# foolwood/SiamMask

Hardware: NVIDIA H100
Metric: search-region frames/sec (127/255 SiamMask-sharp) (higher is better)
Workload: dtype f16x3 (hi+lo split fp16 operands on wgmma, f32 accumulate; f32 CUDA-core xcorr/refine)

## Files before the change

siammask_b200/csrc/conv_gemm_sm90.cu:

```cuda
#include "common.cuh"
#include "ptx.cuh"

#include <cstdlib>
#include <cstring>
#include <mutex>
#include <unordered_map>

namespace smk {

namespace {

constexpr int BLOCK_M = 128;
constexpr int WG_ROWS = 64;
constexpr int CIN_GRAIN = 64;
constexpr int MMA_K = 16;
constexpr int SMEM_LIMIT = 227 * 1024;
constexpr int NUM_CONSUMER_WARPS = 8;
constexpr int NUM_THREADS = 128 + 32 * NUM_CONSUMER_WARPS;
constexpr int PRODUCER_REGS = 40;
constexpr int CONSUMER_REGS = 232;

template <int BLOCK_N, int NSPLIT>
struct Cfg {
  static constexpr int STAGING_BYTES = WG_ROWS * BLOCK_N * 4;
  static constexpr int RING_BYTES = SMEM_LIMIT - 2048 - 2 * STAGING_BYTES;
  static constexpr int stage_bytes(int bk) { return NSPLIT * (BLOCK_M + BLOCK_N) * bk * 2; }
  static constexpr int BLOCK_K = RING_BYTES / stage_bytes(64) >= 3 ? 64 : 32;
  static constexpr int SW = BLOCK_K * 2;
  static constexpr int A_TILE_BYTES = BLOCK_M * BLOCK_K * 2;
  static constexpr int B_TILE_BYTES = BLOCK_N * BLOCK_K * 2;
  static constexpr int STAGE_BYTES = NSPLIT * (A_TILE_BYTES + B_TILE_BYTES);
  static constexpr int RAW_STAGES = RING_BYTES / STAGE_BYTES;
  static constexpr int STAGES = RAW_STAGES > 6 ? 6 : RAW_STAGES;
  static constexpr int SMEM_BYTES = STAGES * STAGE_BYTES + 2 * STAGING_BYTES + 1024  + 256 ;
  static constexpr int ACC = BLOCK_N / 2;
  static constexpr int H_BOX = BLOCK_N < 64 ? BLOCK_N : 64;
  static constexpr int F_BOX = BLOCK_N < 32 ? BLOCK_N : 32;
  static constexpr int H_PLANE = WG_ROWS * BLOCK_N * 2;
  static_assert(STAGES >= 3, "pipeline needs at least three stages");
  static_assert(BLOCK_N % 16 == 0 && BLOCK_N >= 16 && BLOCK_N <= 128, "N tile (register accumulators)");
  static_assert(STAGE_BYTES % 1024 == 0 && B_TILE_BYTES % 1024 == 0, "stage parts stay 1024-aligned (swizzle atoms)");
  static_assert(SMEM_BYTES <= SMEM_LIMIT, "shared memory budget");
};

__device__ __forceinline__ int m_block(const GemmParams& p, int tile) {
  const int mb = tile / p.n_tiles;
  return p.reverse_m ? p.m_tiles - 1 - mb : mb;
}

template <int SPAN>
__device__ __forceinline__ uint32_t swizzle(uint32_t o) {
  return o ^ (((o >> 7) & (SPAN / 16 - 1)) << 4);
}

__device__ __forceinline__ void named_barrier_sync(int id, int threads) {
  asm volatile("bar.sync %0, %1;" ::"r"(id), "r"(threads) : "memory");
}

template <int BLOCK_N, int NSPLIT>
__global__ void __launch_bounds__(NUM_THREADS, 1) conv_gemm_kernel(const __grid_constant__ GemmParams p) {
  using C = Cfg<BLOCK_N, NSPLIT>;
  constexpr int STAGES = C::STAGES;
  constexpr int BLOCK_K = C::BLOCK_K;
  constexpr int A_TILE_BYTES = C::A_TILE_BYTES;

  extern __shared__ uint8_t smem_raw[];
  uint8_t* smem = smem_raw + ((1024u - (smem_u32(smem_raw) & 1023u)) & 1023u);
  uint8_t* staging = smem + STAGES * C::STAGE_BYTES;
  uint64_t* full_bar = reinterpret_cast<uint64_t*>(staging + 2 * C::STAGING_BYTES);
  uint64_t* empty_bar = full_bar + STAGES;
  uint64_t* free_bar = empty_bar + STAGES;
  uint64_t* res_bar = free_bar + 2;

  const int warp = __shfl_sync(0xffffffffu, (int)(threadIdx.x >> 5), 0);
  const int lane = threadIdx.x & 31;
  const int num_tiles = p.m_tiles * p.n_tiles;

  if (threadIdx.x == 0) {
    for (int i = 0; i < NSPLIT; ++i) {
      for (int sgi = 0; sgi < p.nseg; ++sgi) tma_prefetch_desc(&p.seg[sgi].tmA[i]);
      tma_prefetch_desc(&p.tmB[i]);
    }
    for (int s = 0; s < STAGES; ++s) {
      mbar_init(&full_bar[s], 1);
      mbar_init(&empty_bar[s], NUM_CONSUMER_WARPS);
    }
    for (int w = 0; w < 2; ++w) {
      mbar_init(&free_bar[w], 1);
      mbar_init(&res_bar[w], 1);
    }
    fence_barrier_init();
  }
  __syncthreads();

  if (warp < 4) {
    setmaxnreg_dec<PRODUCER_REGS>();
    if (warp != 0) return;
    const bool leader = elect_one();
    int stage = 0;
    uint32_t phase = 0;
    uint32_t iter = 0;
    for (int tile = blockIdx.x; tile < num_tiles; tile += gridDim.x, ++iter) {
      const int m0 = m_block(p, tile) * BLOCK_M;
      const int n0 = (tile % p.n_tiles) * BLOCK_N;
      const int q = m0 % p.Wo;
      const int t = m0 / p.Wo;
      const int pq = t % p.Ho;
      const int nb = t / p.Ho;
      for (int sgi = 0; sgi < p.nseg; ++sgi) {
        const GemmSegment& sg = p.seg[sgi];
        const int wb = q * sg.stride - sg.pad;
        const int hb = pq * sg.stride - sg.pad;
#pragma unroll 1
        for (int kb = 0; kb < sg.num_kb; ++kb) {
          mbar_wait(&empty_bar[stage], phase ^ 1);
          if (leader) mbar_arrive_expect_tx(&full_bar[stage], C::STAGE_BYTES);
          uint8_t* st = smem + stage * C::STAGE_BYTES;
          const int tap = kb / sg.cblks;
          const int c0 = (kb - tap * sg.cblks) * BLOCK_K;
#pragma unroll
          for (int s = 0; s < NSPLIT; ++s) {
            uint8_t* a_dst = st + s * A_TILE_BYTES;
            if (leader) {
              if (sg.mode == 0) {
                tma_load_2d(a_dst, &sg.tmA[s], &full_bar[stage], c0, m0);
              } else {
                const int r = tap / sg.KW;
                const int sx = tap - r * sg.KW;
                tma_load_im2col_4d(a_dst, &sg.tmA[s], &full_bar[stage], c0, wb, hb, nb,
                                   static_cast<uint16_t>(sx * sg.dil), static_cast<uint16_t>(r * sg.dil));
              }
              tma_load_2d(st + NSPLIT * A_TILE_BYTES + s * C::B_TILE_BYTES, &p.tmB[s], &full_bar[stage],
                          sg.b_col0 + kb * BLOCK_K, n0);
            }
          }
          __syncwarp();
          if (++stage == STAGES) { stage = 0; phase ^= 1; }
        }
      }
      if (p.has_res) {
#pragma unroll 1
        for (int w = 0; w < 2; ++w) {
          mbar_wait(&free_bar[w], iter & 1);
          const int r0 = m0 + w * WG_ROWS;
          if (leader) {
            mbar_arrive_expect_tx(&res_bar[w], r0 < p.M ? NSPLIT * C::H_PLANE : 0);
            if (r0 < p.M) {
              uint8_t* dst = staging + w * C::STAGING_BYTES;
#pragma unroll
              for (int s = 0; s < NSPLIT; ++s)
#pragma unroll
                for (int b = 0; b < BLOCK_N / C::H_BOX; ++b)
                  tma_load_2d(dst + s * C::H_PLANE + b * (WG_ROWS * C::H_BOX * 2), &p.tmR[s], &res_bar[w],
                              n0 + b * C::H_BOX, r0);
            }
          }
          __syncwarp();
        }
      }
    }
    return;
  }

  setmaxnreg_inc<CONSUMER_REGS>();
  const int wg = (warp >> 2) - 1;
  const int wl = warp & 3;
  const bool store_thread = wl == 0 && lane == 0;
  const Epilogue& ep = p.ep;
  const int HoWo = p.Ho * p.Wo;
  uint8_t* my_staging = staging + wg * C::STAGING_BYTES;
  float acc[C::ACC];
  float acc2[C::ACC];
  int stage = 0;
  uint32_t phase = 0;
  uint32_t iter = 0;
  for (int tile = blockIdx.x; tile < num_tiles; tile += gridDim.x, ++iter) {
#pragma unroll
    for (int i = 0; i < C::ACC; ++i) { acc[i] = 0.f; acc2[i] = 0.f; }
    int prev = -1;
    for (int sgi = 0; sgi < p.nseg; ++sgi) {
      const int nkb = p.seg[sgi].num_kb;
#pragma unroll 1
      for (int kb = 0; kb < nkb; ++kb) {
        mbar_wait(&full_bar[stage], phase);
        const uint32_t a_hi = smem_u32(smem + stage * C::STAGE_BYTES) + wg * (WG_ROWS * BLOCK_K * 2);
        const uint32_t b_hi = smem_u32(smem + stage * C::STAGE_BYTES) + NSPLIT * A_TILE_BYTES;
        const uint64_t da_hi0 = wgmma_desc_kmajor<C::SW>(a_hi);
        const uint64_t db_hi0 = wgmma_desc_kmajor<C::SW>(b_hi);
        const uint64_t da_lo0 = wgmma_desc_kmajor<C::SW>(a_hi + A_TILE_BYTES);
        const uint64_t db_lo0 = wgmma_desc_kmajor<C::SW>(b_hi + C::B_TILE_BYTES);
        wgmma_fence();
#pragma unroll
        for (int k = 0; k < BLOCK_K / MMA_K; ++k) {
          const uint64_t kadd = static_cast<uint64_t>(k * MMA_K * 2 / 16);
          wgmma_f16<BLOCK_N>(acc, da_hi0 + kadd, db_hi0 + kadd);
          if constexpr (NSPLIT == 2) {
            wgmma_f16<BLOCK_N>(acc2, da_hi0 + kadd, db_lo0 + kadd);
            wgmma_f16<BLOCK_N>(acc2, da_lo0 + kadd, db_hi0 + kadd);
          }
        }
        wgmma_commit();
        wgmma_wait<1>();
        if (prev >= 0) {
          __syncwarp();
          if (lane == 0) mbar_arrive(&empty_bar[prev]);
        } else if (store_thread) {
          tma_store_wait_read<0>();
          mbar_arrive(&free_bar[wg]);
        }
        prev = stage;
        if (++stage == STAGES) { stage = 0; phase ^= 1; }
      }
    }
    wgmma_wait<0>();
    fence_regs(acc);
    if constexpr (NSPLIT == 2) fence_regs(acc2);
    __syncwarp();
    if (lane == 0) mbar_arrive(&empty_bar[prev]);

    const int m0 = m_block(p, tile) * BLOCK_M + wg * WG_ROWS;
    const int n0 = (tile % p.n_tiles) * BLOCK_N;
    const int rl = wl * 16 + (lane >> 2);
    const int cl = 2 * (lane & 3);
    if (ep.out_mode == OUT_NCHW_F32) {
#pragma unroll
      for (int h = 0; h < 2; ++h) {
        const int m = m0 + rl + 8 * h;
        if (m >= p.M) continue;
        const int b = m / HoWo;
        const int hw = m - b * HoWo;
#pragma unroll
        for (int j = 0; j < BLOCK_N / 8; ++j) {
          const int n = n0 + cl + 8 * j;
          float v0 = acc[4 * j + 2 * h], v1 = acc[4 * j + 2 * h + 1];
          if constexpr (NSPLIT == 2) {
            v0 += acc2[4 * j + 2 * h];
            v1 += acc2[4 * j + 2 * h + 1];
          }
          const float2 al = __ldg(reinterpret_cast<const float2*>(ep.alpha + n));
          const float2 be = __ldg(reinterpret_cast<const float2*>(ep.beta + n));
          v0 = fmaf(v0, al.x, be.x);
          v1 = fmaf(v1, al.y, be.y);
          if (ep.relu) {
            v0 = fmaxf(v0, 0.f);
            v1 = fmaxf(v1, 0.f);
          }
          if (n < p.Cout) {
            float* dst = ep.out_f32 + (static_cast<size_t>(b) * p.Cout + n) * HoWo + hw;
            __stcs(dst, v0);
            if (n + 1 < p.Cout) __stcs(dst + HoWo, v1);
          }
        }
      }
      continue;
    }

    mbar_wait(p.has_res ? &res_bar[wg] : &free_bar[wg], iter & 1);
    const bool split = ep.out_mode == OUT_NHWC_SPLIT;
    const bool two_planes = ep.out_lo != nullptr;
    float amax = 0.f;
#pragma unroll
    for (int h = 0; h < 2; ++h) {
      const int r = rl + 8 * h;
      const bool row_in = m0 + r < p.M;
#pragma unroll
      for (int j = 0; j < BLOCK_N / 8; ++j) {
        const int c = cl + 8 * j;
        const int n = n0 + c;
        float v0 = acc[4 * j + 2 * h], v1 = acc[4 * j + 2 * h + 1];
        if constexpr (NSPLIT == 2) {
          v0 += acc2[4 * j + 2 * h];
          v1 += acc2[4 * j + 2 * h + 1];
        }
        const float2 al = __ldg(reinterpret_cast<const float2*>(ep.alpha + n));
        const float2 be = __ldg(reinterpret_cast<const float2*>(ep.beta + n));
        v0 = fmaf(v0, al.x, be.x);
        v1 = fmaf(v1, al.y, be.y);
        const uint32_t oh = (c / C::H_BOX) * (WG_ROWS * C::H_BOX * 2) +
                            swizzle<C::H_BOX * 2>(r * (C::H_BOX * 2) + (c % C::H_BOX) * 2);
        if (p.has_res) {
          float2 f = __half22float2(*reinterpret_cast<const __half2*>(my_staging + oh));
          if constexpr (NSPLIT == 2) {
            const float2 l = __half22float2(*reinterpret_cast<const __half2*>(my_staging + C::H_PLANE + oh));
            f.x += l.x;
            f.y += l.y;
          }
          v0 += f.x * ep.res_scale;
          v1 += f.y * ep.res_scale;
        }
        if (ep.relu) {
          v0 = fmaxf(v0, 0.f);
          v1 = fmaxf(v1, 0.f);
        }
        if (split) {
          if (row_in) amax = fmaxf(amax, fmaxf(fabsf(v0), fabsf(v1)));
          const __half2 hv = __floats2half2_rn(v0, v1);
          const float2 hf = __half22float2(hv);
          *reinterpret_cast<__half2*>(my_staging + oh) = hv;
          if (two_planes)
            *reinterpret_cast<__half2*>(my_staging + C::H_PLANE + oh) = __floats2half2_rn(v0 - hf.x, v1 - hf.y);
        } else {
          const uint32_t of = (c / C::F_BOX) * (WG_ROWS * C::F_BOX * 4) +
                              swizzle<C::F_BOX * 4>(r * (C::F_BOX * 4) + (c % C::F_BOX) * 4);
          *reinterpret_cast<float2*>(my_staging + of) = make_float2(v0, v1);
        }
      }
    }
    fence_proxy_async();
    named_barrier_sync(1 + wg, 128);
    if (store_thread && m0 < p.M) {
      if (split) {
        for (int s = 0; s < (two_planes ? 2 : 1); ++s)
#pragma unroll
          for (int b = 0; b < BLOCK_N / C::H_BOX; ++b)
            tma_store_2d(&p.tmO[s], my_staging + s * C::H_PLANE + b * (WG_ROWS * C::H_BOX * 2), n0 + b * C::H_BOX, m0);
      } else {
#pragma unroll
        for (int b = 0; b < BLOCK_N / C::F_BOX; ++b)
          tma_store_2d(&p.tmO[0], my_staging + b * (WG_ROWS * C::F_BOX * 4), n0 + b * C::F_BOX, m0);
      }
      tma_store_commit();
    }
    if (split) flag_if_out_of_range(amax, ep.ovf);
  }
  if (store_thread) tma_store_wait_all();
}

using EncodeTiledFn = CUresult (*)(CUtensorMap*, CUtensorMapDataType, cuuint32_t, void*, const cuuint64_t*,
                                   const cuuint64_t*, const cuuint32_t*, const cuuint32_t*, CUtensorMapInterleave,
                                   CUtensorMapSwizzle, CUtensorMapL2promotion, CUtensorMapFloatOOBfill);
using EncodeIm2colFn = CUresult (*)(CUtensorMap*, CUtensorMapDataType, cuuint32_t, void*, const cuuint64_t*,
                                    const cuuint64_t*, const int*, const int*, cuuint32_t, cuuint32_t,
                                    const cuuint32_t*, CUtensorMapInterleave, CUtensorMapSwizzle,
                                    CUtensorMapL2promotion, CUtensorMapFloatOOBfill);

struct DriverApi {
  EncodeTiledFn tiled = nullptr;
  EncodeIm2colFn im2col = nullptr;
  int driver_version = 0;
};

const DriverApi& driver_api() {
  static DriverApi api;
  static std::once_flag once;
  std::call_once(once, [] {
    void* fn = nullptr;
    cudaDriverEntryPointQueryResult q;
    SMK_CUDA(cudaGetDriverEntryPoint("cuTensorMapEncodeTiled", &fn, cudaEnableDefault, &q));
    SMK_CHECK(fn != nullptr && q == cudaDriverEntryPointSuccess, "cuTensorMapEncodeTiled not available");
    api.tiled = reinterpret_cast<EncodeTiledFn>(fn);
    fn = nullptr;
    SMK_CUDA(cudaGetDriverEntryPoint("cuTensorMapEncodeIm2col", &fn, cudaEnableDefault, &q));
    SMK_CHECK(fn != nullptr && q == cudaDriverEntryPointSuccess, "cuTensorMapEncodeIm2col not available");
    api.im2col = reinterpret_cast<EncodeIm2colFn>(fn);
    SMK_CUDA(cudaDriverGetVersion(&api.driver_version));
  });
  return api;
}

struct MapKey {
  uint64_t v[16];
  bool operator==(const MapKey& o) const { return std::memcmp(v, o.v, sizeof v) == 0; }
};
struct MapKeyHash {
  size_t operator()(const MapKey& k) const {
    uint64_t h = 0x9E3779B97F4A7C15ull;
    for (uint64_t x : k.v) { h ^= x + 0x9E3779B97F4A7C15ull + (h << 6) + (h >> 2); }
    return (size_t)h;
  }
};
template <typename F>
CUtensorMap cached_map(const MapKey& key, F&& encode) {
  static std::mutex mu;
  static std::unordered_map<MapKey, CUtensorMap, MapKeyHash> cache;
  int dev = 0;
  cudaGetDevice(&dev);
  MapKey k = key;
  k.v[15] = (uint64_t)dev;
  std::lock_guard<std::mutex> lock(mu);
  auto it = cache.find(k);
  if (it != cache.end()) return it->second;
  if (cache.size() > 65536) cache.clear();
  CUtensorMap m = encode();
  cache.emplace(k, m);
  return m;
}

CUtensorMap make_map_2d_raw(const __half* base, uint64_t inner, uint64_t outer, uint32_t box_inner, uint32_t box_outer) {
  CUtensorMap m;
  cuuint64_t dims[2] = {inner, outer};
  cuuint64_t strides[1] = {inner * sizeof(__half)};
  cuuint32_t box[2] = {box_inner, box_outer};
  cuuint32_t estr[2] = {1, 1};
  const CUtensorMapSwizzle sw = box_inner == 64 ? CU_TENSOR_MAP_SWIZZLE_128B : CU_TENSOR_MAP_SWIZZLE_64B;
  CUresult r = driver_api().tiled(&m, CU_TENSOR_MAP_DATA_TYPE_FLOAT16, 2, const_cast<__half*>(base), dims, strides,
                                  box, estr, CU_TENSOR_MAP_INTERLEAVE_NONE, sw,
                                  CU_TENSOR_MAP_L2_PROMOTION_L2_256B, CU_TENSOR_MAP_FLOAT_OOB_FILL_NONE);
  SMK_CHECK(r == CUDA_SUCCESS, "cuTensorMapEncodeTiled failed, code " + std::to_string((int)r));
  return m;
}

CUtensorMap make_map_2d(const __half* base, uint64_t inner, uint64_t outer, uint32_t box_inner, uint32_t box_outer) {
  MapKey k{};
  k.v[0] = 1; k.v[1] = (uint64_t)base; k.v[2] = inner; k.v[3] = outer; k.v[4] = box_inner; k.v[5] = box_outer;
  return cached_map(k, [&] { return make_map_2d_raw(base, inner, outer, box_inner, box_outer); });
}

CUtensorMap make_map_im2col_raw(const __half* base, const Act& in, const ConvGeom& g, int bk) {
  CUtensorMap m;
  cuuint64_t dims[4] = {(cuuint64_t)in.C, (cuuint64_t)in.W, (cuuint64_t)in.H, (cuuint64_t)in.B};
  cuuint64_t strides[3] = {(cuuint64_t)in.C * 2, (cuuint64_t)in.W * in.C * 2, (cuuint64_t)in.H * in.W * in.C * 2};
  int lower[2] = {-g.pad, -g.pad};
  int upper[2] = {g.pad - (g.KW - 1) * g.dil, g.pad - (g.KH - 1) * g.dil};
  cuuint32_t estr[4] = {1, (cuuint32_t)g.stride, (cuuint32_t)g.stride, 1};
  const DriverApi& api = driver_api();
  CUresult r = api.im2col(&m, CU_TENSOR_MAP_DATA_TYPE_FLOAT16, 4, const_cast<__half*>(base), dims, strides, lower,
                          upper, bk, BLOCK_M, estr, CU_TENSOR_MAP_INTERLEAVE_NONE,
                          bk == 64 ? CU_TENSOR_MAP_SWIZZLE_128B : CU_TENSOR_MAP_SWIZZLE_64B,
                          CU_TENSOR_MAP_L2_PROMOTION_L2_256B, CU_TENSOR_MAP_FLOAT_OOB_FILL_NONE);
  SMK_CHECK(r == CUDA_SUCCESS, "cuTensorMapEncodeIm2col failed, code " + std::to_string((int)r));
  if (api.driver_version <= 13010 && in.numel() * sizeof(__half) < 131072)
    reinterpret_cast<uint64_t*>(&m)[1] &= ~(1ull << 21);
  return m;
}

CUtensorMap make_map_im2col(const __half* base, const Act& in, const ConvGeom& g, int bk) {
  MapKey k{};
  k.v[0] = 3; k.v[1] = (uint64_t)base;
  k.v[2] = ((uint64_t)in.B << 32) | (uint32_t)in.H; k.v[3] = ((uint64_t)in.W << 32) | (uint32_t)in.C;
  k.v[4] = ((uint64_t)g.KH << 32) | (uint32_t)g.KW; k.v[5] = ((uint64_t)g.stride << 32) | (uint32_t)g.pad;
  k.v[6] = ((uint64_t)g.dil << 32) | (uint32_t)bk;
  return cached_map(k, [&] { return make_map_im2col_raw(base, in, g, bk); });
}

}

static CUtensorMap make_map_2d_any_raw(const __half* base, uint64_t inner, uint64_t outer, uint32_t box_inner, uint32_t box_outer,
                            int swizzle_bytes) {
  CUtensorMap m;
  cuuint64_t dims[2] = {inner, outer};
  cuuint64_t strides[1] = {inner * sizeof(__half)};
  cuuint32_t box[2] = {box_inner, box_outer};
  cuuint32_t estr[2] = {1, 1};
  const CUtensorMapSwizzle sw = swizzle_bytes == 128 ? CU_TENSOR_MAP_SWIZZLE_128B
                                : swizzle_bytes == 64 ? CU_TENSOR_MAP_SWIZZLE_64B : CU_TENSOR_MAP_SWIZZLE_32B;
  CUresult r = driver_api().tiled(&m, CU_TENSOR_MAP_DATA_TYPE_FLOAT16, 2, const_cast<__half*>(base), dims, strides,
                                  box, estr, CU_TENSOR_MAP_INTERLEAVE_NONE, sw, CU_TENSOR_MAP_L2_PROMOTION_L2_128B,
                                  CU_TENSOR_MAP_FLOAT_OOB_FILL_NONE);
  SMK_CHECK(r == CUDA_SUCCESS, "cuTensorMapEncodeTiled failed, code " + std::to_string((int)r));
  return m;
}

CUtensorMap make_map_2d_any(const __half* base, uint64_t inner, uint64_t outer, uint32_t box_inner, uint32_t box_outer,
                            int swizzle_bytes) {
  MapKey k{};
  k.v[0] = 5; k.v[1] = (uint64_t)base; k.v[2] = inner; k.v[3] = outer; k.v[4] = box_inner; k.v[5] = box_outer;
  k.v[6] = (uint64_t)swizzle_bytes;
  return cached_map(k, [&] { return make_map_2d_any_raw(base, inner, outer, box_inner, box_outer, swizzle_bytes); });
}

static CUtensorMap make_map_tiled_nd_raw(const __half* base, int rank, const uint64_t* dims,
                                         const uint64_t* strides_bytes, const uint32_t* box, int swizzle_bytes) {
  SMK_CHECK(rank >= 2 && rank <= 5, "tensor map rank");
  CUtensorMap m;
  cuuint64_t d[5], sb[4];
  cuuint32_t bx[5], es[5];
  for (int i = 0; i < rank; ++i) { d[i] = dims[i]; bx[i] = box[i]; es[i] = 1; }
  for (int i = 0; i + 1 < rank; ++i) sb[i] = strides_bytes[i];
  const CUtensorMapSwizzle sw = swizzle_bytes == 128 ? CU_TENSOR_MAP_SWIZZLE_128B
                                : swizzle_bytes == 64 ? CU_TENSOR_MAP_SWIZZLE_64B
                                : swizzle_bytes == 32 ? CU_TENSOR_MAP_SWIZZLE_32B : CU_TENSOR_MAP_SWIZZLE_NONE;
  CUresult r = driver_api().tiled(&m, CU_TENSOR_MAP_DATA_TYPE_FLOAT16, (cuuint32_t)rank, const_cast<__half*>(base), d, sb,
                                  bx, es, CU_TENSOR_MAP_INTERLEAVE_NONE, sw, CU_TENSOR_MAP_L2_PROMOTION_L2_256B,
                                  CU_TENSOR_MAP_FLOAT_OOB_FILL_NONE);
  SMK_CHECK(r == CUDA_SUCCESS, "cuTensorMapEncodeTiled (nd) failed, code " + std::to_string((int)r));
  return m;
}

CUtensorMap make_map_tiled_nd(const __half* base, int rank, const uint64_t* dims, const uint64_t* strides_bytes,
                              const uint32_t* box, int swizzle_bytes) {
  SMK_CHECK(rank >= 2 && rank <= 5, "tensor map rank");
  MapKey k{};
  k.v[0] = 4 | ((uint64_t)rank << 8) | ((uint64_t)swizzle_bytes << 16);
  k.v[1] = (uint64_t)base;
  for (int i = 0; i < rank; ++i) k.v[2 + i] = dims[i] | ((uint64_t)box[i] << 40);
  for (int i = 0; i + 1 < rank; ++i) k.v[7 + i] = strides_bytes[i];
  return cached_map(k, [&] { return make_map_tiled_nd_raw(base, rank, dims, strides_bytes, box, swizzle_bytes); });
}

bool gemm_conv_supported(const ConvGeom& g) { return g.Cin % CIN_GRAIN == 0 && g.Cout >= 1; }

int gemm_cout_pad(int cout) {
  if (cout <= 16) return 16;
  if (cout <= 32) return 32;
  if (cout <= 64) return 64;
  if (cout <= 128) return 128;
  return (cout + 255) / 256 * 256;
}

static CUtensorMap make_map_2d_f32(const float* base, uint64_t inner, uint64_t outer, uint32_t box_inner,
                                   uint32_t box_outer, int swizzle_bytes) {
  MapKey k{};
  k.v[0] = 6; k.v[1] = (uint64_t)base; k.v[2] = inner; k.v[3] = outer; k.v[4] = box_inner; k.v[5] = box_outer;
  k.v[6] = (uint64_t)swizzle_bytes;
  return cached_map(k, [&] {
    CUtensorMap m;
    cuuint64_t dims[2] = {inner, outer};
    cuuint64_t strides[1] = {inner * sizeof(float)};
    cuuint32_t box[2] = {box_inner, box_outer};
    cuuint32_t estr[2] = {1, 1};
    const CUtensorMapSwizzle sw = swizzle_bytes == 128 ? CU_TENSOR_MAP_SWIZZLE_128B
                                  : swizzle_bytes == 64 ? CU_TENSOR_MAP_SWIZZLE_64B : CU_TENSOR_MAP_SWIZZLE_32B;
    CUresult r = driver_api().tiled(&m, CU_TENSOR_MAP_DATA_TYPE_FLOAT32, 2, const_cast<float*>(base), dims, strides,
                                    box, estr, CU_TENSOR_MAP_INTERLEAVE_NONE, sw, CU_TENSOR_MAP_L2_PROMOTION_L2_128B,
                                    CU_TENSOR_MAP_FLOAT_OOB_FILL_NONE);
    SMK_CHECK(r == CUDA_SUCCESS, "cuTensorMapEncodeTiled (f32) failed, code " + std::to_string((int)r));
    return m;
  });
}

template <int BLOCK_N, int NSPLIT>
static void launch_cfg(GemmParams& p, const GemmInput* convs, const __half* w_hi, const __half* w_lo, int cout_pad,
                       int w_ld, int num_sms, cudaStream_t st) {
  using C = Cfg<BLOCK_N, NSPLIT>;
  constexpr int bk = C::BLOCK_K;
  for (int i = 0; i < p.nseg; ++i) {
    const ConvGeom& g = convs[i].g;
    const Act& in = convs[i].in;
    GemmSegment& sg = p.seg[i];
    sg.cblks = g.Cin / bk;
    sg.num_kb = g.KH * g.KW * sg.cblks;
    for (int s = 0; s < NSPLIT; ++s) {
      const __half* a = s == 0 ? in.hi : in.lo;
      sg.tmA[s] = sg.mode == 0 ? make_map_2d(a, g.Cin, (uint64_t)in.M(), bk, BLOCK_M) : make_map_im2col(a, in, g, bk);
    }
    if (NSPLIT == 1) sg.tmA[1] = sg.tmA[0];
  }
  if (p.nseg == 1) p.seg[1] = p.seg[0];
  for (int s = 0; s < NSPLIT; ++s) p.tmB[s] = make_map_2d(s == 0 ? w_hi : w_lo, (uint64_t)w_ld, cout_pad, bk, BLOCK_N);
  if (NSPLIT == 1) p.tmB[1] = p.tmB[0];

  auto kern = conv_gemm_kernel<BLOCK_N, NSPLIT>;
  static unsigned long long attr_done = 0;
  ensure_dynamic_smem(kern, C::SMEM_BYTES, attr_done);
  const int tiles = p.m_tiles * p.n_tiles;
  const int grid = tiles < num_sms ? tiles : num_sms;
  kern<<<grid, NUM_THREADS, C::SMEM_BYTES, st>>>(p);
  SMK_CUDA(cudaGetLastError());
}

void launch_gemm_conv(const Act& in, const ConvGeom& g, const __half* w_hi, const __half* w_lo, int cout_pad,
                      const Epilogue& ep, int nsplit, int num_sms, cudaStream_t st) {
  GemmInput gi{in, g, 0};
  launch_gemm_multi(&gi, 1, nullptr, w_hi, w_lo, cout_pad, g.KH * g.KW * g.Cin, ep, nsplit, num_sms, st);
}

void launch_gemm_multi(const GemmInput* convs, int nconv, const Act* residual, const __half* w_hi,
                       const __half* w_lo, int cout_pad, int w_ld, const Epilogue& ep, int nsplit, int num_sms,
                       cudaStream_t st, bool reverse_m) {
  SMK_CHECK(nconv >= 1 && nconv <= 2, "1 or 2 convolution segments");
  const ConvGeom& g0 = convs[0].g;
  const Act& in0 = convs[0].in;
  const int Ho = g0.out_size(in0.H), Wo = g0.out_size(in0.W);
  GemmParams p;
  std::memset(&p, 0, sizeof p);
  p.M = in0.B * Ho * Wo;
  p.Cout = g0.Cout;
  p.Ho = Ho;
  p.Wo = Wo;
  const int block_n = cout_pad < 128 ? cout_pad : 128;
  SMK_CHECK(cout_pad % block_n == 0, "cout_pad must be a multiple of the N tile");
  if (ep.out_mode != OUT_NCHW_F32) SMK_CHECK(g0.Cout == cout_pad, "NHWC outputs need Cout to match the padded tile width");
  p.n_tiles = cout_pad / block_n;
  p.m_tiles = (p.M + BLOCK_M - 1) / BLOCK_M;
  p.reverse_m = reverse_m ? 1 : 0;
  p.nseg = nconv;
  for (int i = 0; i < nconv; ++i) {
    const ConvGeom& g = convs[i].g;
    const Act& in = convs[i].in;
    SMK_CHECK(gemm_conv_supported(g), "Cin must be a multiple of 64 for the tensor-core conv");
    SMK_CHECK(in.C == g.Cin && g.Cout == g0.Cout && in.B == in0.B, "segment channels/batch mismatch");
    SMK_CHECK(g.out_size(in.H) == Ho && g.out_size(in.W) == Wo, "segments must produce the same output size");
    SMK_CHECK(nsplit == 1 || (in.lo != nullptr && w_lo != nullptr), "exact mode needs lo planes");
    GemmSegment& sg = p.seg[i];
    sg.KW = g.KW;
    sg.stride = g.stride;
    sg.pad = g.pad;
    sg.dil = g.dil;
    sg.mode = (g.KH == 1 && g.KW == 1 && g.stride == 1 && g.pad == 0) ? 0 : 1;
    sg.b_col0 = convs[i].w_col0;
    SMK_CHECK(sg.b_col0 % 64 == 0 && sg.b_col0 + g.KH * g.KW * g.Cin <= w_ld, "weight column range");
  }
  const uint32_t hbox = block_n < 64 ? block_n : 64, fbox = block_n < 32 ? block_n : 32;
  auto aligned = [](const void* q) { return (reinterpret_cast<uintptr_t>(q) & 15) == 0; };
  if (ep.out_mode == OUT_NHWC_SPLIT) {
    SMK_CHECK(aligned(ep.out_hi) && (ep.out_lo == nullptr || aligned(ep.out_lo)), "NHWC output planes 16-byte aligned");
    for (int s = 0; s < (ep.out_lo != nullptr ? 2 : 1); ++s)
      p.tmO[s] = make_map_2d_any(s == 0 ? ep.out_hi : ep.out_lo, (uint64_t)p.Cout, (uint64_t)p.M, hbox, 64, hbox * 2);
  } else if (ep.out_mode == OUT_NHWC_F32) {
    SMK_CHECK(aligned(ep.out_f32), "NHWC fp32 output 16-byte aligned");
    p.tmO[0] = make_map_2d_f32(ep.out_f32, (uint64_t)p.Cout, (uint64_t)p.M, fbox, 64, fbox * 4);
  }
  if (residual != nullptr) {
    SMK_CHECK(ep.out_mode == OUT_NHWC_SPLIT, "a residual needs an NHWC split-plane output");
    SMK_CHECK(residual->C == g0.Cout && residual->M() == p.M, "residual shape");
    SMK_CHECK(nsplit == 1 || residual->lo != nullptr, "exact mode residual needs both planes");
    SMK_CHECK(aligned(residual->hi) && (nsplit == 1 || aligned(residual->lo)), "residual planes 16-byte aligned");
    p.has_res = 1;
    for (int s = 0; s < nsplit; ++s)
      p.tmR[s] = make_map_2d_any(s == 0 ? residual->hi : residual->lo, (uint64_t)p.Cout, (uint64_t)p.M, hbox, 64,
                                 hbox * 2);
  }
  p.ep = ep;

#define SMK_DISPATCH(BN)                                                                         \
  case BN:                                                                                       \
    if (nsplit == 2) launch_cfg<BN, 2>(p, convs, w_hi, w_lo, cout_pad, w_ld, num_sms, st);       \
    else launch_cfg<BN, 1>(p, convs, w_hi, w_lo, cout_pad, w_ld, num_sms, st);                   \
    break;
  switch (block_n) {
    SMK_DISPATCH(16)
    SMK_DISPATCH(32)
    SMK_DISPATCH(64)
    SMK_DISPATCH(128)
    default: SMK_CHECK(false, "unsupported N tile");
  }
#undef SMK_DISPATCH
}

}
```

Baseline: 4658.

## Offload NCHW f32 epilogue stores to idle producer warps via swizzled staging

```diff
diff --git a/siammask_b200/csrc/conv_gemm_sm90.cu b/siammask_b200/csrc/conv_gemm_sm90.cu
--- a/siammask_b200/csrc/conv_gemm_sm90.cu
+++ b/siammask_b200/csrc/conv_gemm_sm90.cu
@@ -53,6 +53,10 @@
   return o ^ (((o >> 7) & (SPAN / 16 - 1)) << 4);
 }
 
+__device__ __forceinline__ uint32_t nchw_staging_index(int c, int r) {
+  return c * WG_ROWS + (r ^ (((c >> 1) & 3) << 3));
+}
+
 __device__ __forceinline__ void named_barrier_sync(int id, int threads) {
   asm volatile("bar.sync %0, %1;" ::"r"(id), "r"(threads) : "memory");
 }
@@ -71,6 +75,9 @@
   uint64_t* empty_bar = full_bar + STAGES;
   uint64_t* free_bar = empty_bar + STAGES;
   uint64_t* res_bar = free_bar + 2;
+  uint64_t* stg_full = res_bar + 2;
+  uint64_t* stg_free = stg_full + 2;
+  static_assert((2 * STAGES + 8) * sizeof(uint64_t) <= 256, "barriers fit their reserved bytes (Cfg::SMEM_BYTES)");
 
   const int warp = __shfl_sync(0xffffffffu, (int)(threadIdx.x >> 5), 0);
   const int lane = threadIdx.x & 31;
@@ -88,6 +95,8 @@
     for (int w = 0; w < 2; ++w) {
       mbar_init(&free_bar[w], 1);
       mbar_init(&res_bar[w], 1);
+      mbar_init(&stg_full[w], 4);
+      mbar_init(&stg_free[w], 3);
     }
     fence_barrier_init();
   }
@@ -95,7 +104,59 @@
 
   if (warp < 4) {
     setmaxnreg_dec<PRODUCER_REGS>();
-    if (warp != 0) return;
+    if (warp != 0) {
+      if (p.ep.out_mode != OUT_NCHW_F32) return;
+      const int sw = warp - 1;
+      const int HoWo = p.Ho * p.Wo;
+      const Epilogue& ep = p.ep;
+      const float* const stg[2] = {reinterpret_cast<const float*>(staging),
+                                   reinterpret_cast<const float*>(staging + C::STAGING_BYTES)};
+      uint32_t iter = 0;
+      for (int tile = blockIdx.x; tile < num_tiles; tile += gridDim.x, ++iter) {
+        const int n0 = (tile % p.n_tiles) * BLOCK_N;
+        const int nend = min(BLOCK_N, p.Cout - n0);
+        const int m0 = m_block(p, tile) * BLOCK_M;
+        float* dst[4];
+        bool row_in[4];
+#pragma unroll
+        for (int q = 0; q < 4; ++q) {
+          const int m = m0 + lane + 32 * q;
+          row_in[q] = m < p.M;
+          const int b = row_in[q] ? m / HoWo : 0;
+          const int hw = row_in[q] ? m - b * HoWo : 0;
+          dst[q] = ep.out_f32 + (static_cast<size_t>(b) * p.Cout + n0 + sw) * HoWo + hw;
+        }
+        const size_t step = static_cast<size_t>(3) * HoWo;
+        float alk[2], bek[2];
+#pragma unroll
+        for (int r = 0; r < 2; ++r) {
+          const int c = sw + 3 * (lane + 32 * r);
+          alk[r] = c < nend ? __ldg(ep.alpha + n0 + c) : 0.f;
+          bek[r] = c < nend ? __ldg(ep.beta + n0 + c) : 0.f;
+        }
+        mbar_wait(&stg_full[0], iter & 1);
+        mbar_wait(&stg_full[1], iter & 1);
+#pragma unroll 2
+        for (int c = sw, k = 0; c < nend; c += 3, ++k) {
+          const float al = __shfl_sync(0xffffffffu, k < 32 ? alk[0] : alk[1], k & 31);
+          const float be = __shfl_sync(0xffffffffu, k < 32 ? bek[0] : bek[1], k & 31);
+          const uint32_t i = nchw_staging_index(c, lane);
+#pragma unroll
+          for (int q = 0; q < 4; ++q) {
+            float v = fmaf(stg[q >> 1][i + 32 * (q & 1)], al, be);
+            if (ep.relu) v = fmaxf(v, 0.f);
+            if (row_in[q]) __stcs(dst[q], v);
+            dst[q] += step;
+          }
+        }
+        __syncwarp();
+        if (lane == 0) {
+          mbar_arrive(&stg_free[0]);
+          mbar_arrive(&stg_free[1]);
+        }
+      }
+      return;
+    }
     const bool leader = elect_one();
     int stage = 0;
     uint32_t phase = 0;
@@ -167,7 +228,6 @@
   const int wl = warp & 3;
   const bool store_thread = wl == 0 && lane == 0;
   const Epilogue& ep = p.ep;
-  const int HoWo = p.Ho * p.Wo;
   uint8_t* my_staging = staging + wg * C::STAGING_BYTES;
   float acc[C::ACC];
   float acc2[C::ACC];
@@ -223,35 +283,23 @@
     const int rl = wl * 16 + (lane >> 2);
     const int cl = 2 * (lane & 3);
     if (ep.out_mode == OUT_NCHW_F32) {
+      mbar_wait(&stg_free[wg], (iter & 1) ^ 1);
 #pragma unroll
       for (int h = 0; h < 2; ++h) {
-        const int m = m0 + rl + 8 * h;
-        if (m >= p.M) continue;
-        const int b = m / HoWo;
-        const int hw = m - b * HoWo;
+        float* stg = reinterpret_cast<float*>(my_staging) + nchw_staging_index(cl, rl + 8 * h);
 #pragma unroll
         for (int j = 0; j < BLOCK_N / 8; ++j) {
-          const int n = n0 + cl + 8 * j;
           float v0 = acc[4 * j + 2 * h], v1 = acc[4 * j + 2 * h + 1];
           if constexpr (NSPLIT == 2) {
             v0 += acc2[4 * j + 2 * h];
             v1 += acc2[4 * j + 2 * h + 1];
           }
-          const float2 al = __ldg(reinterpret_cast<const float2*>(ep.alpha + n));
-          const float2 be = __ldg(reinterpret_cast<const float2*>(ep.beta + n));
-          v0 = fmaf(v0, al.x, be.x);
-          v1 = fmaf(v1, al.y, be.y);
-          if (ep.relu) {
-            v0 = fmaxf(v0, 0.f);
-            v1 = fmaxf(v1, 0.f);
-          }
-          if (n < p.Cout) {
-            float* dst = ep.out_f32 + (static_cast<size_t>(b) * p.Cout + n) * HoWo + hw;
-            __stcs(dst, v0);
-            if (n + 1 < p.Cout) __stcs(dst + HoWo, v1);
-          }
+          stg[(8 * j) * WG_ROWS] = v0;
+          stg[(8 * j + 1) * WG_ROWS] = v1;
         }
       }
+      __syncwarp();
+      if (lane == 0) mbar_arrive(&stg_full[wg]);
       continue;
     }
 
```

New measurement: 4759 (median of 6 runs). 2.2% higher.
